# swami1995/diff-qp-mpc

Hardware: AMD Instinct MI355X
Metric: QPs/sec (fwd+bwd), batch=4096 n=3 m=3 T=5 (higher is better)
Workload: dtype f64; 1 GPU; random dense QP family R (SURVEY 8d), configs[0] shape at the BASELINE metric batch: B=4096/GPU nz=30 nineq=30 neq=15; global_batch=4096, n_state=3, n_ctrl=3, T=5, parallelism=batch-shard x1, termination=batch (the reference's batch-coupled rule, parity-safe)

## Files before the change

### diff-qp-mpc_amd/csrc/dqp_r16_prims.h

```cpp
#ifndef DQP_R16_PRIMS_H_
#define DQP_R16_PRIMS_H_
#include <hip/hip_runtime.h>
#include <math.h>

#include "dqp_common.h"

namespace dqp {
namespace r16 {

template <int CTRL> __device__ __forceinline__ double dppd(double v)
{
    return __builtin_amdgcn_update_dpp(v, v, CTRL, 0xf, 0xf, true);
}

__device__ __forceinline__ double rb(double v, int k)
{
    switch (k & 15) {
    case 0: return dppd<0x150>(v);   case 1: return dppd<0x151>(v);
    case 2: return dppd<0x152>(v);   case 3: return dppd<0x153>(v);
    case 4: return dppd<0x154>(v);   case 5: return dppd<0x155>(v);
    case 6: return dppd<0x156>(v);   case 7: return dppd<0x157>(v);
    case 8: return dppd<0x158>(v);   case 9: return dppd<0x159>(v);
    case 10: return dppd<0x15a>(v);  case 11: return dppd<0x15b>(v);
    case 12: return dppd<0x15c>(v);  case 13: return dppd<0x15d>(v);
// ... 297 lines not shown
#pragma unroll
    for (int k = N - 1; k >= 0; --k) {
        const int sk = k >> 4, lk = k & 15;
        const double xk = rb(b[sk] * rdu[sk], lk);
#pragma unroll
        for (int s = 0; s < S; ++s) {
            if (16 * s > k) continue;
            if (16 * s + 15 < k) b[s] = fma(-T[s][k], xk, b[s]);
            else b[s] = fma(-mask_hi(T[s][k], r < lk), xk, b[s]);
        }
    }
#pragma unroll
    for (int s = 0; s < S; ++s) b[s] *= rdu[s];
}

template <int S, int N>
__device__ __forceinline__ void lu_solve(const double (&T)[S][N], const double (&rdu)[S],
                                         double (&b)[S], int r)
{
#pragma unroll
    for (int k = 0; k < N - 1; ++k) {
        const int lk = k & 15;
        const double bk = BC(b, k);
#pragma unroll
        for (int s = 0; s < S; ++s) {
            if (16 * s + 15 <= k) continue;
            if (16 * s > k) b[s] = fma(-T[s][k], bk, b[s]);
            else b[s] = fma(-mask_hi(T[s][k], r > lk), bk, b[s]);
        }
    }
    lu_solve_U<S, N>(T, rdu, b, r);
}

template <int S, int N>
__device__ __forceinline__ void lu_rows_rhs(double (&T)[S][N], double (&rdu)[S], double (&b)[S], int r)
{
    lu_rows_impl<S, N, true, DQP_LU_LOOKAHEAD != 0>(T, rdu, b, r);
}

template <int S, int N, bool FOLD>
__device__ __forceinline__ void lu_factor_solve(double (&T)[S][N], double (&rdu)[S], double (&b)[S], int r)
{
    if (FOLD) {
        lu_rows_rhs<S, N>(T, rdu, b, r);
        lu_solve_U<S, N>(T, rdu, b, r);
    } else {
        lu_rows<S, N>(T, rdu, r);
        lu_solve<S, N>(T, rdu, b, r);
    }
}

template <int S, int N>
__device__ __forceinline__ void trsv_rows(const double (&L)[S][N], const double (&rd)[S],
                                          double (&b)[S], int r)
{
#pragma unroll
    for (int k = 0; k < N; ++k) {
        const int sk = k >> 4, lk = k & 15;
        const double yk = rb(b[sk] * rd[sk], lk);
#pragma unroll
        for (int s = 0; s < S; ++s) {
            if (16 * s + 15 < k) continue;
            if (16 * s > k) b[s] = fma(-L[s][k], yk, b[s]);
            else b[s] = (r == lk) ? yk : fma(r > lk ? -L[s][k] : 0.0, yk, b[s]);
        }
    }
}

template <int S, int N>
__device__ __forceinline__ void tri_store(double *P, const double (&L)[S][N], int r, double *dummy)
{
#pragma unroll
    for (int s = 0; s < S; ++s) {
        const int i = r + 16 * s;
#pragma unroll
        for (int j = 0; j < N; ++j) {
            if (j > 16 * s + 15) continue;
            double *dst = (i < N && j <= i) ? P + tri(i) + j : dummy;
            *dst = L[s][j];
        }
    }
}

template <int S, int N>
__device__ __forceinline__ void tri_mv(const double *P, const double (&x)[S], double (&y)[S], int r)
{
#pragma unroll
    for (int s = 0; s < S; ++s) y[s] = 0.0;
#pragma unroll
    for (int j = 0; j < N; ++j) {
        const double xb = BC(x, j);
#pragma unroll
        for (int s = 0; s < S; ++s) {
            if (16 * s + 15 < j) continue;
            const int i = r + 16 * s;
            const int ic = i < N ? i : N - 1;
            const double v = P[tri(ic) + (j <= ic ? j : 0)];
            y[s] = fma(mask_hi(v, j <= i && i < N), xb, y[s]);
        }
    }
}

template <int S, int N>
__device__ __forceinline__ void tri_solve(const double *P, const double (&rd)[S], double (&b)[S], int r)
{
#pragma unroll
    for (int k = 0; k < N; ++k) {
        const int sk = k >> 4, lk = k & 15;
        const double yk = rb(b[sk] * rd[sk], lk);
#pragma unroll
        for (int s = 0; s < S; ++s) {
            if (16 * s + 15 < k) continue;
            const int i = r + 16 * s;
            const int ic = i < N ? i : N - 1;
            const double v = P[tri(ic) + (k <= ic ? k : 0)];
            if (16 * s > k) b[s] = fma((i < N) ? -v : 0.0, yk, b[s]);
            else b[s] = (r == lk) ? yk : fma((r > lk && i < N) ? -v : 0.0, yk, b[s]);
        }
    }
}

template <int S, int N>
__device__ __forceinline__ void tri_solve_T(const double *P, const double (&rd)[S], double (&b)[S], int r)
{
#pragma unroll
    for (int j = N - 1; j >= 0; --j) {
        const int sj = j >> 4, lj = j & 15;
        double part = 0.0;
#pragma unroll
        for (int s = 0; s < S; ++s) {
            if (16 * s + 15 <= j) continue;
            const int i = r + 16 * s;
            const int ic = i < N ? i : N - 1;
            const double v = P[tri(ic) + (j <= ic ? j : 0)];
            part = fma((i > j && i < N) ? v : 0.0, b[s], part);
        }
        const double tot = row_sum(part);
        if (r == lj) b[sj] = (b[sj] - tot) * rd[sj];
    }
}

template <int S>
__device__ __forceinline__ void vec_put(double *P, const double (&v)[S], int n, int r, double *dummy)
{
#pragma unroll
    for (int s = 0; s < S; ++s) {
        const int i = r + 16 * s;
        double *dst = i < n ? P + i : dummy;
        *dst = v[s];
    }
}
template <int S>
__device__ __forceinline__ void vec_get(const double *P, double (&v)[S], int n, int r)
{
#pragma unroll
    for (int s = 0; s < S; ++s) {
        const int i = r + 16 * s;
        const double x = P[i < n ? i : n - 1];
        v[s] = i < n ? x : 0.0;
    }
}

template <int S, int NC, bool V2>
__device__ __forceinline__ void load_rows_staged(const double *src, int nrows, double (&dst)[S][NC], int r, double *stage)
{
#pragma unroll
    for (int s = 0; s < S; ++s) {
        const int nr = nrows - 16 * s < 16 ? nrows - 16 * s : 16;
        const double *blk = src + 16 * s * NC;
        if (V2 && (reinterpret_cast<unsigned long long>(blk) & 15ull) == 0) {
            const double2 *b2 = reinterpret_cast<const double2 *>(blk);
            double2 *s2 = reinterpret_cast<double2 *>(stage);
#pragma unroll
            for (int k = 0; k < (16 * NC / 2 + 15) / 16; ++k) {
                const int e = r + 16 * k;
                if (e < nr * NC / 2) s2[e] = b2[e];
            }
            if ((nr * NC) & 1) { if (r == 0) stage[nr * NC - 1] = blk[nr * NC - 1]; }
        } else {
#pragma unroll
            for (int k = 0; k < NC; ++k) {
                const int e = r + 16 * k;
                if (e < nr * NC) stage[e] = blk[e];
            }
        }
        __syncthreads();
        const double *row = stage + (r < nr ? r : 0) * NC;
#pragma unroll
        for (int j = 0; j < NC; ++j) dst[s][j] = row[j];
        if (16 * s + 15 >= nrows) {
            const double keep = r < nr ? 1.0 : 0.0;
#pragma unroll
            for (int j = 0; j < NC; ++j) dst[s][j] *= keep;
        }
        __syncthreads();
    }
}

template <int S, int NC>
__device__ __forceinline__ void load_rows(const double *src, int nrows, double (&dst)[S][NC], int r)
{
#pragma unroll
    for (int s = 0; s < S; ++s) {
        const int i = r + 16 * s;
        const double *row = src + (i < nrows ? i : nrows - 1) * NC;
        const double keep = i < nrows ? 1.0 : 0.0;
#pragma unroll
        for (int j = 0; j < NC; ++j) dst[s][j] = row[j];
        if (16 * s + 15 >= nrows) {
#pragma unroll
            for (int j = 0; j < NC; ++j) dst[s][j] *= keep;
        }
    }
}

template <class C>
__device__ __forceinline__ void load_T(double *lds, double (&T)[C::SM][C::M],
                                       const double (&rdiag)[C::SM], const double (&dinv)[C::SM], int r)
// ... 47 lines not shown
```

### diff-qp-mpc_amd/csrc/dqp_r16n.hip

```cpp

#include "dqp_r16_prims.h"

namespace dqp {
namespace r16n {

using namespace dqp::r16;

template <int N_, int M_, int E_> struct Cfg {
    static constexpr int N = N_, M = M_, E = E_, R = N_ - E_;
    static constexpr int SN = slots(N_), SM = slots(M_), SR = slots(N_ - E_);
    static constexpr int SE = E_ > 0 ? slots(E_) : 1, EC = E_ > 0 ? E_ : 1;
    static constexpr bool PARK = slots(N_) >= 3;
#ifndef DQP_R16N_PARK_WU
#define DQP_R16N_PARK_WU 1
#endif
    static constexpr bool PARKWU = PARK || DQP_R16N_PARK_WU;
#ifndef DQP_R16N_PIN_ALL
#define DQP_R16N_PIN_ALL 1
#endif
    static constexpr bool PIN = PARK || DQP_R16N_PIN_ALL;
#ifndef DQP_R16N_SPLIT_ALL
#define DQP_R16N_SPLIT_ALL 0
#endif
    static constexpr bool SPLIT = PARK || DQP_R16N_SPLIT_ALL;
#ifndef DQP_R16N_EARLY_CTX
#define DQP_R16N_EARLY_CTX 1
#endif
    static constexpr bool EARLY = DQP_R16N_EARLY_CTX;
    static constexpr int tailsz = E_ * (N_ - E_) + E_ * (E_ - 1) / 2;
    static constexpr int oLq = 0;
    static constexpr int oTl = tri(N_);
    static constexpr int oR = oTl;
    static constexpr int shared = tailsz > tri(M_) ? tailsz : tri(M_);
    static constexpr int oCp = oTl + shared;
    static constexpr int oHp = oCp + (N_ - E_);
    static constexpr int oQv = oHp + M_;
    static constexpr int oBw = oQv + N_;
    static constexpr int oBs = oBw + (N_ - E_), oBz = oBs + M_, oBc = oBz + M_;
    static constexpr int oDummy = oBc + 2;
    static constexpr int ldsQP = oDummy + 16;
    static constexpr int ldsQPpad = (ldsQP + 1) & ~1;
#ifndef DQP_R16N_STAGED
#define DQP_R16N_STAGED 0
#endif
    static constexpr bool STAGED = DQP_R16N_STAGED && 16 * N_ <= ldsQP - oTl;
    __host__ __device__ static constexpr int toff(int k) { return k * (N_ - E_) + k * (k - 1) / 2; }
    static constexpr int wTl = 0, wLq = tailsz, wG = wLq + tri(N_), wU = wG + M_ * N_;
    static constexpr int wTau = wU + E_ * E_, wRdu = wTau + E_, wRdq = wRdu + E_;
    static constexpr int wXy = wRdq + N_, wPy = wXy + E_, wW1 = wPy + E_, wDl = wW1 + E_;
    static constexpr int wsQP = wDl + 1;
    static constexpr int snapDim = (N_ - E_) + 2 * M_ + 2;
};

#define DQP_PHASE_FENCE() asm volatile("" ::: "memory")
__device__ __forceinline__ void pin(double &x) { asm volatile("" : "+v"(x) : : "memory"); }
__device__ __forceinline__ const double *relabel(const double *p)
{
    asm volatile("" : "+v"(p));
    return p;
}

template <class C> struct State {
    double Gh[C::SM][C::N];
    double LqZ[C::SN][C::R];
    double Ah[C::SE][C::N];
    double tau[C::SE];
    double rdu1[C::SE];
    double xy[C::SE];
    double py[C::SE];
    double w1[C::SE];
    double rdq[C::SN];
    double rdiag[C::SM];
    int status;
};

template <class C>
__device__ __forceinline__ void shift_down(const double (&vn)[C::SN], double (&ve)[C::SE], int r)
{
#pragma unroll
    for (int s = 0; s < C::SE; ++s) ve[s] = 0.0;
#pragma unroll
    for (int e = 0; e < C::E; ++e) {
        const double t = BC(vn, C::R + e);
        if (r == (e & 15)) ve[e >> 4] = t;
    }
}
template <class C>
__device__ __forceinline__ void shift_up(const double (&ve)[C::SE], double (&vn)[C::SN], int r)
{
#pragma unroll
    for (int e = 0; e < C::E; ++e) {
        const double t = BC(ve, e);
        if (r == ((C::R + e) & 15)) vn[(C::R + e) >> 4] = t;
    }
}

template <class C>
__device__ __forceinline__ void reflect1(const double *lds, const double (&tau)[C::SE],
                                         double (&v)[C::SN], int k, int r)
{
    const int ck = C::R + k;
    const double *tl = lds + C::oTl + C::toff(k);
    double ud[C::SN], dot = 0.0;
#pragma unroll
    for (int s = 0; s < C::SN; ++s) {
        if (16 * s > ck) { ud[s] = 0.0; continue; }
        const int c = r + 16 * s;
        const double t = tl[c < ck ? c : 0];
        ud[s] = c < ck ? t : (c == ck ? 1.0 : 0.0);
        dot = fma(ud[s], v[s], dot);
    }
    const double tw = BC(tau, k) * row_sum(dot);
#pragma unroll
    for (int s = 0; s < C::SN; ++s)
        if (16 * s <= ck) v[s] = fma(-tw, ud[s], v[s]);
}
template <class C>
__device__ __forceinline__ void apply_QfT(const double *lds, const double (&tau)[C::SE],
                                          double (&v)[C::SN], int r)
{
#pragma unroll
    for (int k = C::E - 1; k >= 0; --k) reflect1<C>(lds, tau, v, k, r);
}
template <class C>
__device__ __forceinline__ void apply_Qf(const double *lds, const double (&tau)[C::SE],
                                         double (&v)[C::SN], int r)
{
#pragma unroll
    for (int k = 0; k < C::E; ++k) reflect1<C>(lds, tau, v, k, r);
}

template <class C>
__device__ __forceinline__ void solve_UT(const State<C> &st, double (&t)[C::SE], int r)
{
#pragma unroll
    for (int j = 0; j < C::E; ++j) {
        const int sj = j >> 4, lj = j & 15;
        double part = 0.0;
#pragma unroll
        for (int s = 0; s < C::SE; ++s) {
            if (16 * s >= j) continue;
            const int k = r + 16 * s;
            part = fma(k < j ? st.Ah[s][C::R + j] : 0.0, t[s], part);
        }
        const double tot = row_sum(part);
        if (r == lj) t[sj] = (t[sj] - tot) * st.rdu1[sj];
    }
}

template <class C>
__device__ __forceinline__ void mul_Gz(const State<C> &st, const double (&v)[C::SR], double (&y)[C::SM])
{
#pragma unroll
    for (int s = 0; s < C::SM; ++s) y[s] = 0.0;
#pragma unroll
    for (int t = 0; t < C::R; ++t) {
        const double vb = BC(v, t);
#pragma unroll
        for (int s = 0; s < C::SM; ++s) y[s] = fma(st.Gh[s][t], vb, y[s]);
    }
}
template <class C>
__device__ __forceinline__ void mul_GzT(const State<C> &st, const double (&v)[C::SM], double (&y)[C::SR], int r)
{
#pragma unroll
    for (int g = 0; g < C::SR; ++g) {
        double p[16];
#pragma unroll
        for (int k = 0; k < 16; ++k) {
            const int c = 16 * g + k;
            if (c < C::R) {
                double a = st.Gh[0][c < C::R ? c : 0] * v[0];
#pragma unroll
                for (int s = 1; s < C::SM; ++s) a = fma(st.Gh[s][c < C::R ? c : 0], v[s], a);
                p[k] = a;
            } else {
                p[k] = 0.0;
            }
        }
        y[g] = reduce_scatter16(p, r);
    }
}
template <class C>
__device__ __forceinline__ void mul_WT(const State<C> &st, const double (&v)[C::SM], double (&y)[C::SE], int r)
{
#pragma unroll
    for (int g = 0; g < C::SE; ++g) {
        double p[16];
#pragma unroll
        for (int k = 0; k < 16; ++k) {
            const int e = 16 * g + k;
            if (e < C::E) {
                double a = st.Gh[0][C::R + (e < C::E ? e : 0)] * v[0];
#pragma unroll
                for (int s = 1; s < C::SM; ++s) a = fma(st.Gh[s][C::R + (e < C::E ? e : 0)], v[s], a);
                p[k] = a;
            } else {
                p[k] = 0.0;
            }
        }
        y[g] = reduce_scatter16(p, r);
    }
}

template <int S, int NC>
__device__ __forceinline__ void mpc_rows_Q(const KParams &P, long long qp, double (&dst)[S][NC], int r)
{
    const int nt = P.mn + P.mm;
#pragma unroll
    for (int s = 0; s < S; ++s) {
        const int i = r + 16 * s, ic = i < NC ? i : NC - 1;
        const int t = ic / nt, j = ic - t * nt;
        const double *row = P.mC + (((long long)t * P.B + qp) * nt + j) * nt;
// ... 149 lines not shown
        for (int s = 0; s < C::SN; ++s)
#pragma unroll
            for (int c = 0; c < C::R; ++c) a += st.LqZ[s][c];
    }
    if (K >= 15) {
#pragma unroll
        for (int s = 0; s < C::SM; ++s) a += st.rdiag[s];
    }
    return a;
}
#endif

template <class C>
__device__ __forceinline__ void setup(const KParams &P, long long qp, int r, double *lds, State<C> &st)
{
    constexpr int N = C::N, M = C::M, E = C::E, R = C::R;
    constexpr int SN = C::SN, SM = C::SM, SE = C::SE, SR = C::SR;
    double *dummy = lds + C::oDummy + r;
    st.status = DQP_STATUS_OK;
    double p0[SN], h0[SM], b0[SE];
    const bool mpc = P.mC != nullptr;
    if (mpc) {
        const int n = P.mn, m = P.mm, nt = n + m, T = P.mT;
#pragma unroll
        for (int s = 0; s < SN; ++s) {
            const int i = r + 16 * s, ic = i < N ? i : N - 1, t = ic / nt;
            const double v = P.mc[((long long)t * P.B + qp) * nt + (ic - t * nt)];
            p0[s] = i < N ? v : 0.0;
        }
#pragma unroll
        for (int s = 0; s < SM; ++s) {
            const int i = r + 16 * s, k = (i < T * m ? i : i - T * m), kc = k < T * m ? k : 0, t = kc / m, ju = kc - t * m;
            const long long at = qp * mpc_bound_stride_b(P) + t * mpc_bound_stride_t(P) + ju;
            const double v = i < T * m ? P.muu[at] : -P.mul[at];
            h0[s] = i < M ? v : 0.0;
        }
#pragma unroll
        for (int s = 0; s < SE; ++s) {
            const int e = r + 16 * s, ec = e < E ? e : (E > 0 ? E - 1 : 0), t = ec / n, j = ec - t * n;
            const double v = t < T - 1 ? -P.mf[((long long)t * P.B + qp) * n + j] : P.mx0[qp * n + j];
            b0[s] = (E > 0 && e < E) ? v : 0.0;
        }
    } else {
#pragma unroll
        for (int s = 0; s < SN; ++s) p0[s] = (r + 16 * s < N) ? P.p[qp * P.sp + r + 16 * s] : 0.0;
#pragma unroll
        for (int s = 0; s < SM; ++s) h0[s] = (r + 16 * s < M) ? P.h[qp * P.sh + r + 16 * s] : 0.0;
#pragma unroll
        for (int s = 0; s < SE; ++s) b0[s] = (E > 0 && r + 16 * s < E) ? P.b[qp * P.sb + r + 16 * s] : 0.0;
    }
    {
        double Lq[SN][N];
        if (mpc) mpc_rows_Q<SN, N>(P, qp, Lq, r);
        else if (C::STAGED) load_rows_staged<SN, N, (N * N) % 2 == 0>(P.Q + qp * P.sQ, N, Lq, r, lds + C::oTl);
        else load_rows<SN, N>(P.Q + qp * P.sQ, N, Lq, r);
        if (!chol_rows<SN, N>(Lq, st.rdq, r)) st.status = DQP_STATUS_Q_NOT_PD;
        tri_store<SN, N>(lds + C::oLq, Lq, r, dummy);
    }
    __syncthreads();
    if (C::EARLY) {
        double *ws = P.workspace + qp * (long long)C::wsQP;
        lds_to_ctx<tri(N)>(lds + C::oLq, ws + C::wLq, r);
#pragma unroll
        for (int s = 0; s < SN; ++s)
            if (r + 16 * s < N) ws[C::wRdq + r + 16 * s] = st.rdq[s];
    }
    __builtin_amdgcn_sched_barrier(0);
    DQP_PHASE_FENCE();
    STAMP(P, 1);

    if (mpc) {
        if (!C::SPLIT) mpc_rows_G<SM, N>(P, M, st.Gh, r);
        if (E > 0) mpc_rows_A<SE, N>(P, qp, E, st.Ah, r);
    } else {
        if (C::STAGED) {
            if (!C::SPLIT) load_rows_staged<SM, N, (M * N) % 2 == 0>(P.G + qp * P.sG, M, st.Gh, r, lds + C::oTl);
            if (E > 0) load_rows_staged<SE, N, (C::EC * N) % 2 == 0>(P.A + qp * P.sA, E, st.Ah, r, lds + C::oTl);
        } else {
            if (!C::SPLIT) load_rows<SM, N>(P.G + qp * P.sG, M, st.Gh, r);
            if (E > 0) load_rows<SE, N>(P.A + qp * P.sA, E, st.Ah, r);
        }
    }
    {
        const double *Lp = lds + C::oLq;
#pragma unroll
        for (int j = 0; j < N; ++j) {
#pragma unroll
            for (int k = 0; k < j; ++k) {
                const double ljk = Lp[tri(j) + k];
                if (!C::SPLIT) {
#pragma unroll
                    for (int s = 0; s < SM; ++s) st.Gh[s][j] = fma(-st.Gh[s][k], ljk, st.Gh[s][j]);
                }
                if (E > 0) {
#pragma unroll
                    for (int s = 0; s < SE; ++s) st.Ah[s][j] = fma(-st.Ah[s][k], ljk, st.Ah[s][j]);
                }
            }
            const double rj = BC(st.rdq, j);
            if (!C::SPLIT) {
#pragma unroll
                for (int s = 0; s < SM; ++s) st.Gh[s][j] *= rj;
            }
            if (E > 0) {
#pragma unroll
                for (int s = 0; s < SE; ++s) st.Ah[s][j] *= rj;
            }
            if (C::PIN) {
#pragma unroll
                for (int s = 0; s < SE; ++s) pin(st.Ah[s][j]);
                if (!C::SPLIT) {
#pragma unroll
                    for (int s = 0; s < SM; ++s) pin(st.Gh[s][j]);
                }
            }
            __builtin_amdgcn_sched_barrier(0);
        }
    }
    __builtin_amdgcn_sched_barrier(0);
    DQP_PHASE_FENCE();
    STAMP(P, 2);

#pragma unroll
    for (int s = 0; s < SE; ++s) { st.tau[s] = 0.0; st.rdu1[s] = 0.0; st.xy[s] = 0.0; st.py[s] = 0.0; st.w1[s] = 0.0; }

    if (E > 0) {
        double nmax = 0.0;
#pragma unroll
        for (int k = E - 1; k >= 0; --k) {
            const int sk = k >> 4, lk = k & 15, ck = R + k;
#ifdef DQP_STAMPS_C
            if (k < 15) { STAMPC(P, k); }
#endif
            double u[N];
            double nrm2 = 0.0;
#pragma unroll
            for (int c = 0; c <= ck; ++c) {
                u[c] = rb(st.Ah[sk][c], lk);
                nrm2 = fma(u[c], u[c], nrm2);
            }
            if (!(nrm2 > 1e-26 * nmax)) { if (st.status == DQP_STATUS_OK) st.status = DQP_STATUS_A_RANK_DEF; nrm2 = 1.0; }
            nmax = fmax(nmax, nrm2);
            const double vk = u[ck];
            const double alpha = -copysign(sqrt(nrm2), vk);
            const double uck = vk - alpha;
            const double iu = frcp(uck);
            const double tauk = uck * uck * frcp(nrm2 - alpha * vk);
            double *tl = lds + C::oTl + C::toff(k);
            if (C::PIN) {
#pragma unroll
                for (int c = 0; c < ck; ++c) u[c] *= iu;
                if (r == 0) {
#pragma unroll
                    for (int c = 0; c < ck; ++c) tl[c] = u[c];
                }
            } else {
#pragma unroll
                for (int c = 0; c < ck; ++c) {
                    u[c] *= iu;
                    double *dst = (r == 0) ? tl + c : dummy;
                    *dst = u[c];
                }
            }
            if (r == lk) { st.tau[sk] = tauk; st.rdu1[sk] = frcp(alpha); }
#pragma unroll
            for (int s = 0; s < SE; ++s) {
                if (16 * s > k) continue;
                double w = st.Ah[s][ck];
#pragma unroll
                for (int c = 0; c < ck; ++c) w = fma(st.Ah[s][c], u[c], w);
                double tw = tauk * w;
                if (16 * s + 15 >= k) tw = (r + 16 * s < k) ? tw : 0.0;
// ... 30 lines not shown
        __builtin_amdgcn_sched_barrier(0);
        if (C::EARLY) {
            double *ws = P.workspace + qp * (long long)C::wsQP;
            lds_to_ctx<C::tailsz>(lds + C::oTl, ws + C::wTl, r);
        }
        DQP_PHASE_FENCE();

        {
            double b[SE];
#pragma unroll
            for (int s = 0; s < SE; ++s) b[s] = b0[s];
#pragma unroll
            for (int j = E - 1; j >= 0; --j) {
                const int sj = j >> 4, lj = j & 15;
                const double xj = rb(b[sj] * st.rdu1[sj], lj);
#pragma unroll
                for (int s = 0; s < SE; ++s) {
                    if (16 * s > j) continue;
                    const int k = r + 16 * s;
                    b[s] = (k == j) ? xj : fma(k < j ? -st.Ah[s][R + j] : 0.0, xj, b[s]);
                }
            }
#pragma unroll
            for (int s = 0; s < SE; ++s) st.xy[s] = b[s];
        }
    }
    __builtin_amdgcn_sched_barrier(0);
    DQP_PHASE_FENCE();
    if (C::SPLIT) {
        if (mpc) mpc_rows_G<SM, N>(P, M, st.Gh, r);
        else if (C::STAGED) load_rows_staged<SM, N, (M * N) % 2 == 0>(P.G + qp * P.sG, M, st.Gh, r, lds + C::oTl);
        else load_rows<SM, N>(P.G + qp * P.sG, M, st.Gh, r);
        const double *Lp = relabel(lds + C::oLq);
#pragma unroll
        for (int j = 0; j < N; ++j) {
#pragma unroll
            for (int k = 0; k < j; ++k) {
                const double ljk = Lp[tri(j) + k];
#pragma unroll
                for (int s = 0; s < SM; ++s) st.Gh[s][j] = fma(-st.Gh[s][k], ljk, st.Gh[s][j]);
            }
            const double rj = BC(st.rdq, j);
#pragma unroll
            for (int s = 0; s < SM; ++s) { st.Gh[s][j] *= rj; pin(st.Gh[s][j]); }
            __builtin_amdgcn_sched_barrier(0);
        }
        if (E > 0) {
#pragma unroll
            for (int k = E - 1; k >= 0; --k) {
                const int ck = R + k;
                const double *tl = lds + C::oTl + C::toff(k);
                const double tauk = BC(st.tau, k);
                double w[SM];
#pragma unroll
                for (int s = 0; s < SM; ++s) w[s] = st.Gh[s][ck];
#pragma unroll
                for (int c = 0; c < ck; ++c) {
                    const double uc = tl[c];
#pragma unroll
                    for (int s = 0; s < SM; ++s) w[s] = fma(st.Gh[s][c], uc, w[s]);
                }
#pragma unroll
                for (int s = 0; s < SM; ++s) { w[s] *= tauk; st.Gh[s][ck] -= w[s]; }
#pragma unroll
                for (int c = 0; c < ck; ++c) {
                    const double uc = tl[c];
#pragma unroll
                    for (int s = 0; s < SM; ++s) st.Gh[s][c] = fma(-w[s], uc, st.Gh[s][c]);
                }
#pragma unroll
                for (int s = 0; s < SM; ++s) { pin(st.Gh[s][0]); pin(st.Gh[s][ck]); }
                __builtin_amdgcn_sched_barrier(0);
            }
        }
    }
    __builtin_amdgcn_sched_barrier(0);
    DQP_PHASE_FENCE();
    STAMP(P, 3);

    {
        double ph[SN];
#pragma unroll
        for (int s = 0; s < SN; ++s) ph[s] = p0[s];
        tri_solve<SN, N>(C::SPLIT ? relabel(lds + C::oLq) : lds + C::oLq, st.rdq, ph, r);
        if (E > 0) {
            apply_QfT<C>(lds, st.tau, ph, r);
            shift_down<C>(ph, st.py, r);
        }
#pragma unroll
        for (int s = 0; s < SN; ++s) {
            const int i = r + 16 * s;
            double *dst = i < R ? lds + C::oCp + i : dummy;
            *dst = ph[s];
        }
    }
    {
        double hp[SM];
#pragma unroll
        for (int s = 0; s < SM; ++s) hp[s] = h0[s];
        if (E > 0) {
#pragma unroll
            for (int e = 0; e < E; ++e) {
                const double xb = BC(st.xy, e);
#pragma unroll
                for (int s = 0; s < SM; ++s) hp[s] = fma(-st.Gh[s][R + e], xb, hp[s]);
            }
            double one[SM];
#pragma unroll
            for (int s = 0; s < SM; ++s) one[s] = (r + 16 * s < M) ? 1.0 : 0.0;
            mul_WT<C>(st, one, st.w1, r);
        }
        vec_put<SM>(lds + C::oHp, hp, M, r, dummy);
    }
    __builtin_amdgcn_sched_barrier(0);
    DQP_PHASE_FENCE();
    STAMP(P, 4);

    if (C::EARLY && !C::PARK) park_GU<C>(P.workspace + qp * (long long)C::wsQP, st, r);
    if (E > 0) {
        double *ws = P.workspace + qp * (long long)C::wsQP;
#pragma unroll
        for (int s = 0; s < SE; ++s) {
            const int k = r + 16 * s;
            if (k < E) { ws[C::wXy + k] = st.xy[s]; ws[C::wPy + k] = st.py[s]; ws[C::wW1 + k] = st.w1[s]; }
        }
    }
    if (C::PARKWU && E > 0) {
        if (C::PARK || !C::EARLY) park_GU<C>(P.workspace + qp * (long long)C::wsQP, st, r);
#pragma unroll
        for (int s = 0; s < SM; ++s)
#pragma unroll
            for (int e = 0; e < E; ++e) st.Gh[s][R + e] = 0.0;
#pragma unroll
        for (int s = 0; s < SE; ++s)
#pragma unroll
            for (int c = 0; c < N; ++c) st.Ah[s][c] = 0.0;
        __builtin_amdgcn_sched_barrier(0);
        DQP_PHASE_FENCE();
    }
    {
        double Ld[SN][N];
        const double *Lp = lds + C::oLq;
#pragma unroll
        for (int s = 0; s < SN; ++s) {
            const int i = r + 16 * s, ic = i < N ? i : N - 1;
#pragma unroll
            for (int j = 0; j < N; ++j) {
                if (j > 16 * s + 15) { Ld[s][j] = 0.0; continue; }
                const double v = Lp[tri(ic) + (j <= ic ? j : 0)];
                Ld[s][j] = (j <= i && i < N) ? v : 0.0;
            }
        }
        if (E > 0) {
#pragma unroll
            for (int k = E - 1; k >= 0; --k) {
                const int ck = R + k;
                const double *tl = lds + C::oTl + C::toff(k);
                const double tauk = BC(st.tau, k);
                double w[SN];
#pragma unroll
                for (int s = 0; s < SN; ++s) w[s] = Ld[s][ck];
#pragma unroll
                for (int c = 0; c < ck; ++c) {
                    const double uc = tl[c];
#pragma unroll
                    for (int s = 0; s < SN; ++s) w[s] = fma(Ld[s][c], uc, w[s]);
                }
// ... 31 lines not shown
    __builtin_amdgcn_sched_barrier(0);
    DQP_PHASE_FENCE();
    STAMP(P, 5);

    {
        if (!C::EARLY) {
            double *ws = P.workspace + qp * (long long)C::wsQP;
            lds_to_ctx<C::tailsz>(lds + C::oTl, ws + C::wTl, r);
            lds_to_ctx<tri(N)>(lds + C::oLq, ws + C::wLq, r);
            if (!C::PARKWU) park_GU<C>(ws, st, r);
#pragma unroll
            for (int s = 0; s < SN; ++s)
                if (r + 16 * s < N) ws[C::wRdq + r + 16 * s] = st.rdq[s];
        }
    }
    __syncthreads();
    {
        double *Rp = lds + C::oR;
#pragma unroll
        for (int j = 0; j < M; ++j) {
            const int sj = j >> 4, lj = j & 15;
            double acc[SM];
#pragma unroll
            for (int s = 0; s < SM; ++s) acc[s] = 0.0;
#pragma unroll
            for (int c = 0; c < R; ++c) {
                const double gb = rb(st.Gh[sj][c], lj);
#pragma unroll
                for (int s = 0; s < SM; ++s)
                    if (16 * s + 15 >= j) acc[s] = fma(st.Gh[s][c], gb, acc[s]);
            }
#pragma unroll
            for (int s = 0; s < SM; ++s) {
                if (16 * s + 15 < j) continue;
                const int i = r + 16 * s;
                double *dst = (i < M && j <= i) ? Rp + tri(i) + j : dummy;
                *dst = acc[s];
            }
        }
    }
    __syncthreads();
#pragma unroll
    for (int s = 0; s < SM; ++s) {
        const int i = r + 16 * s;
        const double v = (lds + C::oR)[tri(i < M ? i : M - 1) + (i < M ? i : M - 1)];
        st.rdiag[s] = i < M ? v : 0.0;
    }
    __builtin_amdgcn_sched_barrier(0);
    DQP_PHASE_FENCE();
}

template <class C>
__device__ __forceinline__ double rx_norm2_partial(const State<C> &st, const double *lds,
                                                   const double (&rw)[C::SR], double cc, int r)
{
    double rx[C::SN];
    vec_get<C::SN>(lds + C::oQv, rx, C::N, r);
#pragma unroll
    for (int s = 0; s < C::SN; ++s) rx[s] *= cc;
#pragma unroll
    for (int t = 0; t < C::R; ++t) {
        const double vb = BC(rw, t);
#pragma unroll
        for (int s = 0; s < C::SN; ++s) rx[s] = fma(st.LqZ[s][t], vb, rx[s]);
    }
    double a = 0.0;
#pragma unroll
    for (int s = 0; s < C::SN; ++s) a = fma(rx[s], rx[s], a);
    return a;
}

template <class C>
__device__ __forceinline__ void epilogue(const KParams &P, long long qp, int r, double *lds, State<C> &st,
                                         double bestc, double delta, int iters, double best, bool live,
                                         bool reload_tails)
{
    constexpr int N = C::N, M = C::M, E = C::E, R = C::R;
    constexpr int SN = C::SN, SM = C::SM, SE = C::SE, SR = C::SR;
    bool inM[SM];
#pragma unroll
    for (int s = 0; s < SM; ++s) inM[s] = r + 16 * s < M;
    CtxRegs<C::tailsz> tl;
    if (E > 0 && reload_tails) ctx_fetch<C::tailsz>(P.workspace + qp * (long long)C::wsQP + C::wTl, tl, r);
    __syncthreads();
    if (E > 0 && reload_tails) ctx_stash<C::tailsz>(lds + C::oTl, tl, r);
    __syncthreads();

    double bw[SR], bs[SM], bz[SM];
    vec_get<SR>(lds + C::oBw, bw, R, r);
    vec_get<SM>(lds + C::oBs, bs, M, r);
    vec_get<SM>(lds + C::oBz, bz, M, r);
    double xh[SN];
#pragma unroll
    for (int s = 0; s < SN; ++s) xh[s] = (s < SR && r + 16 * s < R) ? bw[s < SR ? s : 0] : 0.0;
    double yv[SE];
#pragma unroll
    for (int s = 0; s < SE; ++s) yv[s] = 0.0;
    if (E > 0) {
        if (C::PARKWU && reload_tails) unpark_WU<C>(P.workspace + qp * (long long)C::wsQP, st, r);
        shift_up<C>(st.xy, xh, r);
        apply_Qf<C>(lds, st.tau, xh, r);
        double wz[SE];
        mul_WT<C>(st, bz, wz, r);
#pragma unroll
        for (int s = 0; s < SE; ++s)
            yv[s] = (r + 16 * s < E) ? bestc * delta * st.w1[s] - st.xy[s] - st.py[s] - wz[s] : 0.0;
        solve_UT<C>(st, yv, r);
    }
    tri_solve_T<SN, N>(lds + C::oLq, st.rdq, xh, r);
    if (live) {
#pragma unroll
        for (int s = 0; s < SN; ++s)
            if (r + 16 * s < N) P.zhat[qp * N + r + 16 * s] = xh[s];
#pragma unroll
        for (int s = 0; s < SM; ++s)
            if (inM[s]) { P.lam[qp * M + r + 16 * s] = bz[s]; P.slack[qp * M + r + 16 * s] = bs[s]; }
        if (E > 0) {
#pragma unroll
            for (int s = 0; s < SE; ++s)
                if (r + 16 * s < E) P.nu[qp * E + r + 16 * s] = yv[s];
        }
        if (r == 0) {
            if (P.info) { P.info[2 * qp] = st.status; P.info[2 * qp + 1] = iters; }
            if (P.best_resid) P.best_resid[qp] = best;
        }
    }
}

template <class C>
__global__ __launch_bounds__(64) void forward_kernel(KParams P)
{
    constexpr int N = C::N, M = C::M, E = C::E, R = C::R;
    constexpr int SN = C::SN, SM = C::SM, SE = C::SE, SR = C::SR;
    extern __shared__ __attribute__((aligned(16))) double sm[];
    const int lane = threadIdx.x, r = lane & 15, qrow = lane >> 4;
    long long qp = (long long)blockIdx.x * 4 + qrow;
    bool live = qp < P.B;
    if (!live) qp = P.B - 1;
    int maxIter = P.maxIter;
    const bool batch = (P.flags & DQP_FLAG_BATCH_TERMINATION) != 0;
    const bool strict = (P.flags & DQP_FLAG_STRICT_GET_STEP) != 0;
    if (P.cap) {
        const int cap = term_cap<true>(P);
        maxIter = min(maxIter, cap);
        live = live && term_flagged(P, qp, cap);
        if (__builtin_amdgcn_ballot_w64(live) == 0) return;
    }
    double *lds = sm + qrow * C::ldsQPpad;
    double *dummy = lds + C::oDummy + r;

    term_zero_acc(P);
    State<C> st;
    STAMP(P, 0);
    setup<C>(P, qp, r, lds, st);
    STAMP(P, 15);

    bool inM[SM], inR[SR];
#pragma unroll
    for (int s = 0; s < SM; ++s) inM[s] = r + 16 * s < M;
#pragma unroll
    for (int s = 0; s < SR; ++s) inR[s] = r + 16 * s < R;

    double T[SM][M], rdu[SM];
    double w[SR], s_[SM], z[SM];
    double cc = 1.0, delta = 0.0;
    {
        double one[SM], hp[SM], cp[SR], g[SM], gtz[SR];
#pragma unroll
        for (int s = 0; s < SM; ++s) one[s] = inM[s] ? 1.0 : 0.0;
        vec_get<SM>(lds + C::oHp, hp, M, r);
        vec_get<SR>(lds + C::oCp, cp, R, r);
        mul_Gz<C>(st, cp, g);
#pragma unroll
        for (int s = 0; s < SM; ++s) g[s] = inM[s] ? -hp[s] - g[s] : 0.0;
        __builtin_amdgcn_sched_barrier(0);
        factor_T_rhs<C>(lds, T, st.rdiag, one, rdu, g, r);
        __builtin_amdgcn_sched_barrier(0);
        mul_GzT<C>(st, g, gtz, r);
#pragma unroll
        for (int s = 0; s < SR; ++s) w[s] = inR[s] ? -cp[s] - gtz[s] : 0.0;
        double ms = INFINITY, mz = INFINITY;
#pragma unroll
        for (int s = 0; s < SM; ++s) {
            z[s] = inM[s] ? g[s] : 0.0;
            s_[s] = -z[s];
            ms = fmin(ms, inM[s] ? s_[s] : INFINITY);
            mz = fmin(mz, inM[s] ? z[s] : INFINITY);
        }
        ms = row_min(ms); mz = row_min(mz);
#pragma unroll
        for (int s = 0; s < SM; ++s) {
            if (ms < 0.0 && inM[s]) s_[s] -= ms - 1.0;
// ... 205 lines not shown
    const int cap = min(P.maxIter, istar);
    double *lds = sm + qrow * C::ldsQPpad;
    double *dummy = lds + C::oDummy + r;
    State<C> st;
    load_ctx<C>(P, qp, r, lds, st);
    const double *ws = P.workspace + qp * (long long)C::wsQP;
#pragma unroll
    for (int s = 0; s < SE; ++s) {
        const int k = r + 16 * s, kc = k < E ? k : (E > 0 ? E - 1 : 0);
        const double a = ws[C::wXy + kc], b = ws[C::wPy + kc], c = ws[C::wW1 + kc];
        st.xy[s] = (E > 0 && k < E) ? a : 0.0;
        st.py[s] = (E > 0 && k < E) ? b : 0.0;
        st.w1[s] = (E > 0 && k < E) ? c : 0.0;
    }
    const double delta = ws[C::wDl];
    const double2 *h = reinterpret_cast<const double2 *>(P.histIn) + qp;
    double hv[64];
#pragma unroll
    for (int it = 0; it < 64; ++it) hv[it] = h[(long long)(it < cap ? it : 0) * P.B].x;
    double best = hv[0];
    int arg = 0;
#pragma unroll
    for (int it = 1; it < 64; ++it)
        if (it < cap && hv[it] < best) { best = hv[it]; arg = it; }
    const double *sp = P.snap + ((long long)arg * P.B + qp) * C::snapDim;
    double bw[SR], bs[SM], bz[SM];
#pragma unroll
    for (int s = 0; s < SR; ++s) { const int i = r + 16 * s; const double v = sp[i < R ? i : 0]; bw[s] = i < R ? v : 0.0; }
#pragma unroll
    for (int s = 0; s < SM; ++s) {
        const int i = r + 16 * s, ic = i < M ? i : 0;
        const double a = sp[R + ic], b = sp[R + M + ic];
        bs[s] = i < M ? a : 0.0;
        bz[s] = i < M ? b : 0.0;
    }
    const double bestc = sp[R + 2 * M];
    vec_put<SR>(lds + C::oBw, bw, R, r, dummy);
    vec_put<SM>(lds + C::oBs, bs, M, r, dummy);
    vec_put<SM>(lds + C::oBz, bz, M, r, dummy);
    st.status = P.info ? P.info[2 * qp] : DQP_STATUS_OK;
    epilogue<C>(P, qp, r, lds, st, bestc, delta, cap, best, live, false);
}

template <class C>
__global__ __launch_bounds__(64) void backward_kernel(KParams P)
{
    constexpr int N = C::N, M = C::M, E = C::E, R = C::R;
    constexpr int SN = C::SN, SM = C::SM, SE = C::SE, SR = C::SR;
    extern __shared__ __attribute__((aligned(16))) double sm[];
    const int lane = threadIdx.x, r = lane & 15, qrow = lane >> 4;
    long long qp = (long long)blockIdx.x * 4 + qrow;
    const bool live = qp < P.B;
    if (!live) qp = P.B - 1;
    double *lds = sm + qrow * C::ldsQPpad;

    State<C> st;
    load_ctx<C>(P, qp, r, lds, st);
    __syncthreads();

    bool inN[SN], inM[SM], inE[SE];
#pragma unroll
    for (int s = 0; s < SN; ++s) inN[s] = r + 16 * s < N;
#pragma unroll
    for (int s = 0; s < SM; ++s) inM[s] = r + 16 * s < M;
#pragma unroll
    for (int s = 0; s < SE; ++s) inE[s] = r + 16 * s < E;

    double zh[SN], g[SN], lam[SM], dinv[SM], nu[SE];
#pragma unroll
    for (int s = 0; s < SN; ++s) {
        zh[s] = inN[s] ? P.zin[qp * N + r + 16 * s] : 0.0;
        g[s] = inN[s] ? P.gin[qp * N + r + 16 * s] : 0.0;
    }
#pragma unroll
    for (int s = 0; s < SM; ++s) {
        lam[s] = inM[s] ? P.lamin[qp * M + r + 16 * s] : 0.0;
        const double sl = inM[s] ? P.slackin[qp * M + r + 16 * s] : 1.0;
        if (P.flags & DQP_FLAG_DENSE_BACKWARD) dinv[s] = inM[s] ? sl / lam[s] : 0.0;
        else dinv[s] = inM[s] ? fmax(sl, 1e-8) / fmax(lam[s], 1e-8) : 0.0;
    }
#pragma unroll
    for (int s = 0; s < SE; ++s) nu[s] = (E > 0 && inE[s]) ? P.nuin[qp * E + r + 16 * s] : 0.0;

    tri_solve<SN, N>(lds + C::oLq, st.rdq, g, r);
    double gy[SE];
#pragma unroll
    for (int s = 0; s < SE; ++s) gy[s] = 0.0;
    if (E > 0) {
        apply_QfT<C>(lds, st.tau, g, r);
        shift_down<C>(g, gy, r);
    }
    double gz[SR];
#pragma unroll
    for (int s = 0; s < SR; ++s) gz[s] = (r + 16 * s < R) ? g[s] : 0.0;

    double dlam[SM];
    mul_Gz<C>(st, gz, dlam);
#pragma unroll
    for (int s = 0; s < SM; ++s) dlam[s] = -dlam[s];
    __builtin_amdgcn_sched_barrier(0);
    {
        double T[SM][M], rdu[SM];
#pragma unroll
        for (int j = 0; j < M; ++j) {
            const int sj = j >> 4, lj = j & 15;
            double acc[SM];
#pragma unroll
            for (int s = 0; s < SM; ++s) acc[s] = (r + 16 * s == j) ? dinv[s] : 0.0;
#pragma unroll
            for (int c = 0; c < R; ++c) {
                const double gb = rb(st.Gh[sj][c], lj);
#pragma unroll
                for (int s = 0; s < SM; ++s) acc[s] = fma(st.Gh[s][c], gb, acc[s]);
            }
#pragma unroll
            for (int s = 0; s < SM; ++s) T[s][j] = acc[s];
            __builtin_amdgcn_sched_barrier(0);
        }
        lu_factor_solve<SM, M, DQP_LU_FOLD_RHS != 0>(T, rdu, dlam, r);
    }
    __builtin_amdgcn_sched_barrier(0);
    double dxh[SN], dnu[SE];
    {
        double gtd[SR];
        mul_GzT<C>(st, dlam, gtd, r);
#pragma unroll
        for (int s = 0; s < SN; ++s) dxh[s] = (s < SR && r + 16 * s < R) ? -(gz[s < SR ? s : 0] + gtd[s < SR ? s : 0]) : 0.0;
    }
#pragma unroll
    for (int s = 0; s < SE; ++s) dnu[s] = 0.0;
    if (E > 0) {
        apply_Qf<C>(lds, st.tau, dxh, r);
        double wz[SE];
        mul_WT<C>(st, dlam, wz, r);
#pragma unroll
        for (int s = 0; s < SE; ++s) dnu[s] = inE[s] ? -(gy[s] + wz[s]) : 0.0;
        solve_UT<C>(st, dnu, r);
    }
    tri_solve_T<SN, N>(lds + C::oLq, st.rdq, dxh, r);

    if (!live) return;
    if (P.mdc || P.mdC || P.mdF || P.mdf || P.mdx0) {
        const int n = P.mn, m = P.mm, nt = n + m, T = P.mT;
        const long long Bq = P.B;
        int tl[SN], jl[SN];
#pragma unroll
        for (int s = 0; s < SN; ++s) { const int c = r + 16 * s; tl[s] = c / nt; jl[s] = c - tl[s] * nt; }
        if (P.mdc) {
#pragma unroll
            for (int s = 0; s < SN; ++s)
                if (inN[s]) P.mdc[((long long)tl[s] * Bq + qp) * nt + jl[s]] = dxh[s];
        }
        if (P.mdC) {
            int ti = 0, ji = 0;
#pragma unroll
            for (int i = 0; i < N; ++i) {
                const double dxi = BC(dxh, i), zi = BC(zh, i);
#pragma unroll
                for (int s = 0; s < SN; ++s)
                    if (inN[s] && tl[s] == ti)
                        P.mdC[(((long long)ti * Bq + qp) * nt + ji) * nt + jl[s]] = 0.5 * (dxi * zh[s] + zi * dxh[s]);
                if (++ji == nt) { ji = 0; ++ti; }
            }
        }
        if (E > 0) {
            int te = 0, je = 0;
#pragma unroll
            for (int e = 0; e < E; ++e) {
                const double dni = BC(dnu, e), ni = BC(nu, e);
                if (te < T - 1) {
                    if (P.mdF) {
#pragma unroll
                        for (int s = 0; s < SN; ++s)
                            if (inN[s] && tl[s] == te)
                                P.mdF[(((long long)te * Bq + qp) * n + je) * nt + jl[s]] = dni * zh[s] + ni * dxh[s];
                    }
                    if (P.mdf && r == 0) P.mdf[((long long)te * Bq + qp) * n + je] = dni;
                } else if (P.mdx0 && r == 0) {
                    P.mdx0[qp * n + je] = -dni;
                }
                if (++je == n) { je = 0; ++te; }
            }
        }
        if (r == 0 && P.info) { P.info[2 * qp] = st.status; P.info[2 * qp + 1] = 0; }
        return;
    }
#pragma unroll
    for (int s = 0; s < SN; ++s)
        if (P.dp && inN[s]) P.dp[qp * N + r + 16 * s] = dxh[s];
#pragma unroll
    for (int s = 0; s < SM; ++s)
        if (P.dh && inM[s]) P.dh[qp * M + r + 16 * s] = -dlam[s];
    if (E > 0) {
#pragma unroll
        for (int s = 0; s < SE; ++s)
            if (P.db && inE[s]) P.db[qp * E + r + 16 * s] = -dnu[s];
    }
    if (P.dQ) {
        double *o = P.dQ + qp * N * N;
#pragma unroll
        for (int i = 0; i < N; ++i) {
            const double dxi = BC(dxh, i), zi = BC(zh, i);
#pragma unroll
            for (int s = 0; s < SN; ++s)
                if (inN[s]) o[i * N + r + 16 * s] = 0.5 * (dxi * zh[s] + zi * dxh[s]);
        }
    }
    if (P.dG) {
        double *o = P.dG + qp * M * N;
#pragma unroll
        for (int i = 0; i < M; ++i) {
            const double dli = BC(dlam, i), li = BC(lam, i);
#pragma unroll
            for (int s = 0; s < SN; ++s)
                if (inN[s]) o[i * N + r + 16 * s] = dli * zh[s] + li * dxh[s];
        }
    }
    if (P.dA && E > 0) {
        double *o = P.dA + qp * E * N;
#pragma unroll
        for (int i = 0; i < E; ++i) {
            const double dni = BC(dnu, i), ni = BC(nu, i);
// ... 46 lines not shown
```

Baseline: 17.33 million QPs/sec.

## Software-prefetch LDS operands in triangular solves, reflectors and row updates

Adds ring-buffered LDS prefetching to tri_mv, tri_solve and tri_solve_T, so columns several steps ahead are loaded while the current column is used. Applies the same double-buffered prefetch to the Householder reflector chains and to the Lq row stream used in the row-elimination loop. Hoists the bw/bs/bz vector loads ahead of the barriers. The aim is to hide LDS latency in the dependent serial chains, at the cost of more live registers, which could lower occupancy or cause spills. It only applies to configurations without register parking (slots(N) < 3).

```diff
diff --git a/diff-qp-mpc_amd/csrc/dqp_r16_prims.h b/diff-qp-mpc_amd/csrc/dqp_r16_prims.h
--- a/diff-qp-mpc_amd/csrc/dqp_r16_prims.h
+++ b/diff-qp-mpc_amd/csrc/dqp_r16_prims.h
@@ -403,58 +403,164 @@
     }
 }
 
-template <int S, int N>
+#ifndef DQP_LDS_PREFETCH
+#define DQP_LDS_PREFETCH 1
+#endif
+#ifndef DQP_TRI_RING
+#define DQP_TRI_RING 4
+#endif
+#ifndef DQP_PF_TRI
+#define DQP_PF_TRI DQP_LDS_PREFETCH
+#endif
+
+__device__ __forceinline__ void after_reads(double &x) { asm volatile("" : "+v"(x) : : "memory"); }
+
+template <int S, int N>
+__device__ __forceinline__ void tri_col(const double *P, double (&c)[S], int k, int r)
+{
+#pragma unroll
+    for (int s = 0; s < S; ++s) {
+        if (16 * s + 15 < k) { c[s] = 0.0; continue; }
+        const int i = r + 16 * s;
+        const int ic = i < N ? i : N - 1;
+        c[s] = P[tri(ic) + (k <= ic ? k : 0)];
+    }
+}
+
+template <int S> __device__ __forceinline__ void ring_use(double (&c)[S], int k)
+{
+#pragma unroll
+    for (int s = 0; s < S; ++s)
+        if (16 * s + 15 >= k) PIN(c[s]);
+}
+
+template <int S, int N, int D = (DQP_PF_TRI ? DQP_TRI_RING : 0)>
 __device__ __forceinline__ void tri_mv(const double *P, const double (&x)[S], double (&y)[S], int r)
 {
 #pragma unroll
     for (int s = 0; s < S; ++s) y[s] = 0.0;
+    if constexpr (D == 0) {
+#pragma unroll
+        for (int j = 0; j < N; ++j) {
+            const double xb = BC(x, j);
+#pragma unroll
+            for (int s = 0; s < S; ++s) {
+                if (16 * s + 15 < j) continue;
+                const int i = r + 16 * s;
+                const int ic = i < N ? i : N - 1;
+                const double v = P[tri(ic) + (j <= ic ? j : 0)];
+                y[s] = fma(mask_hi(v, j <= i && i < N), xb, y[s]);
+            }
+        }
+        return;
+    }
+    constexpr int DR = D > 0 ? D : 1;
+    double ring[DR][S];
+#pragma unroll
+    for (int j = 0; j < D && j < N; ++j) tri_col<S, N>(P, ring[j], j, r);
 #pragma unroll
     for (int j = 0; j < N; ++j) {
+        double col[S];
+#pragma unroll
+        for (int s = 0; s < S; ++s) col[s] = ring[j % DR][s];
+        if (j + D < N) tri_col<S, N>(P, ring[j % DR], j + D, r);
+        after_reads(y[S - 1]);
+        ring_use<S>(col, j);
         const double xb = BC(x, j);
 #pragma unroll
         for (int s = 0; s < S; ++s) {
             if (16 * s + 15 < j) continue;
             const int i = r + 16 * s;
-            const int ic = i < N ? i : N - 1;
-            const double v = P[tri(ic) + (j <= ic ? j : 0)];
-            y[s] = fma(mask_hi(v, j <= i && i < N), xb, y[s]);
-        }
-    }
-}
-
-template <int S, int N>
+            y[s] = fma(mask_hi(col[s], j <= i && i < N), xb, y[s]);
+        }
+    }
+}
+
+template <int S, int N, int D = (DQP_PF_TRI ? DQP_TRI_RING : 0)>
 __device__ __forceinline__ void tri_solve(const double *P, const double (&rd)[S], double (&b)[S], int r)
 {
+    if constexpr (D == 0) {
+#pragma unroll
+        for (int k = 0; k < N; ++k) {
+            const int sk = k >> 4, lk = k & 15;
+            const double yk = rb(b[sk] * rd[sk], lk);
+#pragma unroll
+            for (int s = 0; s < S; ++s) {
+                if (16 * s + 15 < k) continue;
+                const int i = r + 16 * s;
+                const int ic = i < N ? i : N - 1;
+                const double v = P[tri(ic) + (k <= ic ? k : 0)];
+                if (16 * s > k) b[s] = fma((i < N) ? -v : 0.0, yk, b[s]);
+                else b[s] = (r == lk) ? yk : fma((r > lk && i < N) ? -v : 0.0, yk, b[s]);
+            }
+        }
+        return;
+    }
+    constexpr int DR = D > 0 ? D : 1;
+    double ring[DR][S];
+#pragma unroll
+    for (int k = 0; k < D && k < N; ++k) tri_col<S, N>(P, ring[k], k, r);
 #pragma unroll
     for (int k = 0; k < N; ++k) {
         const int sk = k >> 4, lk = k & 15;
+        double col[S];
+#pragma unroll
+        for (int s = 0; s < S; ++s) col[s] = ring[k % DR][s];
+        if (k + D < N) tri_col<S, N>(P, ring[k % DR], k + D, r);
+        after_reads(b[sk]);
+        ring_use<S>(col, k);
         const double yk = rb(b[sk] * rd[sk], lk);
 #pragma unroll
         for (int s = 0; s < S; ++s) {
             if (16 * s + 15 < k) continue;
             const int i = r + 16 * s;
-            const int ic = i < N ? i : N - 1;
-            const double v = P[tri(ic) + (k <= ic ? k : 0)];
+            const double v = col[s];
             if (16 * s > k) b[s] = fma((i < N) ? -v : 0.0, yk, b[s]);
             else b[s] = (r == lk) ? yk : fma((r > lk && i < N) ? -v : 0.0, yk, b[s]);
         }
     }
 }
 
-template <int S, int N>
+template <int S, int N, int D = (DQP_PF_TRI ? DQP_TRI_RING : 0)>
 __device__ __forceinline__ void tri_solve_T(const double *P, const double (&rd)[S], double (&b)[S], int r)
 {
+    if constexpr (D == 0) {
+#pragma unroll
+        for (int j = N - 1; j >= 0; --j) {
+            const int sj = j >> 4, lj = j & 15;
+            double part = 0.0;
+#pragma unroll
+            for (int s = 0; s < S; ++s) {
+                if (16 * s + 15 <= j) continue;
+                const int i = r + 16 * s;
+                const int ic = i < N ? i : N - 1;
+                const double v = P[tri(ic) + (j <= ic ? j : 0)];
+                part = fma((i > j && i < N) ? v : 0.0, b[s], part);
+            }
+            const double tot = row_sum(part);
+            if (r == lj) b[sj] = (b[sj] - tot) * rd[sj];
+        }
+        return;
+    }
+    constexpr int DR = D > 0 ? D : 1;
+    double ring[DR][S];
+#pragma unroll
+    for (int j = N - 1; j > N - 1 - D && j >= 0; --j) tri_col<S, N>(P, ring[j % DR], j, r);
 #pragma unroll
     for (int j = N - 1; j >= 0; --j) {
         const int sj = j >> 4, lj = j & 15;
+        double col[S];
+#pragma unroll
+        for (int s = 0; s < S; ++s) col[s] = ring[j % DR][s];
+        if (j - D >= 0) tri_col<S, N>(P, ring[j % DR], j - D, r);
+        after_reads(b[S - 1]);
+        ring_use<S>(col, j);
         double part = 0.0;
 #pragma unroll
         for (int s = 0; s < S; ++s) {
             if (16 * s + 15 <= j) continue;
             const int i = r + 16 * s;
-            const int ic = i < N ? i : N - 1;
-            const double v = P[tri(ic) + (j <= ic ? j : 0)];
-            part = fma((i > j && i < N) ? v : 0.0, b[s], part);
+            part = fma((i > j && i < N) ? col[s] : 0.0, b[s], part);
         }
         const double tot = row_sum(part);
         if (r == lj) b[sj] = (b[sj] - tot) * rd[sj];
diff --git a/diff-qp-mpc_amd/csrc/dqp_r16n.hip b/diff-qp-mpc_amd/csrc/dqp_r16n.hip
--- a/diff-qp-mpc_amd/csrc/dqp_r16n.hip
+++ b/diff-qp-mpc_amd/csrc/dqp_r16n.hip
@@ -5,12 +5,25 @@
 namespace r16n {
 
 using namespace dqp::r16;
+
+#ifndef DQP_PF_REFLECT
+#define DQP_PF_REFLECT DQP_LDS_PREFETCH
+#endif
+#ifndef DQP_PF_ROWS
+#define DQP_PF_ROWS DQP_LDS_PREFETCH
+#endif
+#ifndef DQP_PF_HEADS
+#define DQP_PF_HEADS DQP_LDS_PREFETCH
+#endif
 
 template <int N_, int M_, int E_> struct Cfg {
     static constexpr int N = N_, M = M_, E = E_, R = N_ - E_;
     static constexpr int SN = slots(N_), SM = slots(M_), SR = slots(N_ - E_);
     static constexpr int SE = E_ > 0 ? slots(E_) : 1, EC = E_ > 0 ? E_ : 1;
     static constexpr bool PARK = slots(N_) >= 3;
+    static constexpr bool PF = !PARK;
+    static constexpr int RING = (PF && DQP_PF_TRI) ? DQP_TRI_RING : 0;
+    static constexpr bool PF_REFLECT = PF && DQP_PF_REFLECT, PF_ROWS = PF && DQP_PF_ROWS, PF_HEADS = PF && DQP_PF_HEADS;
 #ifndef DQP_R16N_PARK_WU
 #define DQP_R16N_PARK_WU 1
 #endif
@@ -96,6 +109,36 @@
 }
 
 template <class C>
+__device__ __forceinline__ void reflect_fetch(const double *lds, double (&t)[C::SN], int k, int r)
+{
+    const int ck = C::R + k;
+    const double *tl = lds + C::oTl + C::toff(k);
+#pragma unroll
+    for (int s = 0; s < C::SN; ++s) {
+        if (16 * s > ck) { t[s] = 0.0; continue; }
+        const int c = r + 16 * s;
+        t[s] = tl[c < ck ? c : 0];
+    }
+}
+template <class C>
+__device__ __forceinline__ void reflect_apply(const double (&t)[C::SN], const double (&tau)[C::SE],
+                                              double (&v)[C::SN], int k, int r)
+{
+    const int ck = C::R + k;
+    double ud[C::SN], dot = 0.0;
+#pragma unroll
+    for (int s = 0; s < C::SN; ++s) {
+        if (16 * s > ck) { ud[s] = 0.0; continue; }
+        const int c = r + 16 * s;
+        ud[s] = c < ck ? t[s] : (c == ck ? 1.0 : 0.0);
+        dot = fma(ud[s], v[s], dot);
+    }
+    const double tw = BC(tau, k) * row_sum(dot);
+#pragma unroll
+    for (int s = 0; s < C::SN; ++s)
+        if (16 * s <= ck) v[s] = fma(-tw, ud[s], v[s]);
+}
+template <class C>
 __device__ __forceinline__ void reflect1(const double *lds, const double (&tau)[C::SE],
                                          double (&v)[C::SN], int k, int r)
 {
@@ -115,20 +158,64 @@
     for (int s = 0; s < C::SN; ++s)
         if (16 * s <= ck) v[s] = fma(-tw, ud[s], v[s]);
 }
+template <class C, bool PF>
+__device__ __forceinline__ void reflect_chain(const double *lds, const double (&tau)[C::SE],
+                                              double (&v)[C::SN], int k0, int dk, int r)
+{
+    if constexpr (!PF) {
+#pragma unroll
+        for (int n = 0; n < C::E; ++n) reflect1<C>(lds, tau, v, k0 + n * dk, r);
+        return;
+    }
+    double t[2][C::SN];
+    if (C::E > 0) reflect_fetch<C>(lds, t[0], k0, r);
+#pragma unroll
+    for (int n = 0; n < C::E; ++n) {
+        const int k = k0 + n * dk;
+        if (n + 1 < C::E) reflect_fetch<C>(lds, t[(n + 1) & 1], k + dk, r);
+        after_reads(v[0]);
+#pragma unroll
+        for (int s = 0; s < C::SN; ++s)
+            if (16 * s <= C::R + k) PIN(t[n & 1][s]);
+        reflect_apply<C>(t[n & 1], tau, v, k, r);
+    }
+}
 template <class C>
 __device__ __forceinline__ void apply_QfT(const double *lds, const double (&tau)[C::SE],
                                           double (&v)[C::SN], int r)
 {
-#pragma unroll
-    for (int k = C::E - 1; k >= 0; --k) reflect1<C>(lds, tau, v, k, r);
+    reflect_chain<C, C::PF_REFLECT>(lds, tau, v, C::E - 1, -1, r);
 }
 template <class C>
 __device__ __forceinline__ void apply_Qf(const double *lds, const double (&tau)[C::SE],
                                          double (&v)[C::SN], int r)
 {
-#pragma unroll
-    for (int k = 0; k < C::E; ++k) reflect1<C>(lds, tau, v, k, r);
-}
+    reflect_chain<C, C::PF_REFLECT>(lds, tau, v, 0, 1, r);
+}
+
+struct LdsStream {
+    double b[2][8];
+    int q;
+};
+__device__ __forceinline__ void stream_chunk(const double *lds, LdsStream &t, int q)
+{
+#pragma unroll
+    for (int i = 0; i < 8; ++i) t.b[q & 1][i] = lds[8 * q + i];
+}
+__device__ __forceinline__ void stream_open(const double *lds, LdsStream &t, int first, int last)
+{
+    t.q = first >> 3;
+    stream_chunk(lds, t, t.q);
+    if (t.q + 1 <= (last >> 3)) stream_chunk(lds, t, t.q + 1);
+}
+__device__ __forceinline__ bool stream_advance(const double *lds, LdsStream &t, int f, int last)
+{
+    if ((f >> 3) == t.q) return false;
+    t.q = f >> 3;
+    if (t.q + 1 <= (last >> 3)) stream_chunk(lds, t, t.q + 1);
+    return true;
+}
+__device__ __forceinline__ double stream_at(const LdsStream &t, int f) { return t.b[(f >> 3) & 1][f & 7]; }
 
 template <class C>
 __device__ __forceinline__ void solve_UT(const State<C> &st, double (&t)[C::SE], int r)
@@ -444,12 +531,25 @@
         }
     }
     {
+        static_assert(C::oLq == 0, "the Lq stream runs on the LDS array's own chunk grid");
         const double *Lp = lds + C::oLq;
+        constexpr int lastLq = tri(N - 1) + N - 2;
+        LdsStream lq;
+        if (C::PF_ROWS && N > 1) stream_open(Lp, lq, tri(1), lastLq);
 #pragma unroll
         for (int j = 0; j < N; ++j) {
 #pragma unroll
             for (int k = 0; k < j; ++k) {
-                const double ljk = Lp[tri(j) + k];
+                double ljk;
+                if (C::PF_ROWS) {
+                    if (stream_advance(Lp, lq, tri(j) + k, lastLq)) {
+                        if (E > 0) after_reads(st.Ah[0][j]);
+                        else if (!C::SPLIT) after_reads(st.Gh[0][j]);
+                    }
+                    ljk = stream_at(lq, tri(j) + k);
+                } else {
+                    ljk = Lp[tri(j) + k];
+                }
                 if (!C::SPLIT) {
 #pragma unroll
                     for (int s = 0; s < SM; ++s) st.Gh[s][j] = fma(-st.Gh[s][k], ljk, st.Gh[s][j]);
@@ -646,7 +746,7 @@
         double ph[SN];
 #pragma unroll
         for (int s = 0; s < SN; ++s) ph[s] = p0[s];
-        tri_solve<SN, N>(C::SPLIT ? relabel(lds + C::oLq) : lds + C::oLq, st.rdq, ph, r);
+        tri_solve<SN, N, C::RING>(C::SPLIT ? relabel(lds + C::oLq) : lds + C::oLq, st.rdq, ph, r);
         if (E > 0) {
             apply_QfT<C>(lds, st.tau, ph, r);
             shift_down<C>(ph, st.py, r);
@@ -844,14 +944,20 @@
     for (int s = 0; s < SM; ++s) inM[s] = r + 16 * s < M;
     CtxRegs<C::tailsz> tl;
     if (E > 0 && reload_tails) ctx_fetch<C::tailsz>(P.workspace + qp * (long long)C::wsQP + C::wTl, tl, r);
+    double bw[SR], bs[SM], bz[SM];
+    if (C::PF_HEADS) {
+        vec_get<SR>(lds + C::oBw, bw, R, r);
+        vec_get<SM>(lds + C::oBs, bs, M, r);
+        vec_get<SM>(lds + C::oBz, bz, M, r);
+    }
     __syncthreads();
     if (E > 0 && reload_tails) ctx_stash<C::tailsz>(lds + C::oTl, tl, r);
     __syncthreads();
-
-    double bw[SR], bs[SM], bz[SM];
-    vec_get<SR>(lds + C::oBw, bw, R, r);
-    vec_get<SM>(lds + C::oBs, bs, M, r);
-    vec_get<SM>(lds + C::oBz, bz, M, r);
+    if (!C::PF_HEADS) {
+        vec_get<SR>(lds + C::oBw, bw, R, r);
+        vec_get<SM>(lds + C::oBs, bs, M, r);
+        vec_get<SM>(lds + C::oBz, bz, M, r);
+    }
     double xh[SN];
 #pragma unroll
     for (int s = 0; s < SN; ++s) xh[s] = (s < SR && r + 16 * s < R) ? bw[s < SR ? s : 0] : 0.0;
@@ -869,7 +975,7 @@
             yv[s] = (r + 16 * s < E) ? bestc * delta * st.w1[s] - st.xy[s] - st.py[s] - wz[s] : 0.0;
         solve_UT<C>(st, yv, r);
     }
-    tri_solve_T<SN, N>(lds + C::oLq, st.rdq, xh, r);
+    tri_solve_T<SN, N, C::RING>(lds + C::oLq, st.rdq, xh, r);
     if (live) {
 #pragma unroll
         for (int s = 0; s < SN; ++s)
@@ -1241,7 +1347,7 @@
 #pragma unroll
     for (int s = 0; s < SE; ++s) nu[s] = (E > 0 && inE[s]) ? P.nuin[qp * E + r + 16 * s] : 0.0;
 
-    tri_solve<SN, N>(lds + C::oLq, st.rdq, g, r);
+    tri_solve<SN, N, C::RING>(lds + C::oLq, st.rdq, g, r);
     double gy[SE];
 #pragma unroll
     for (int s = 0; s < SE; ++s) gy[s] = 0.0;
@@ -1296,7 +1402,7 @@
         for (int s = 0; s < SE; ++s) dnu[s] = inE[s] ? -(gy[s] + wz[s]) : 0.0;
         solve_UT<C>(st, dnu, r);
     }
-    tri_solve_T<SN, N>(lds + C::oLq, st.rdq, dxh, r);
+    tri_solve_T<SN, N, C::RING>(lds + C::oLq, st.rdq, dxh, r);
 
     if (!live) return;
     if (P.mdc || P.mdC || P.mdF || P.mdf || P.mdx0) {
```

Measured after the change: 17.97 million QPs/sec (median of 6 runs). +3.7%, better.
